# ebeauce/Seismic_BPMF

Hardware: AMD Instinct MI355X
Metric: million network-CC-samples/s (matched filter) (higher is better)
Workload: dtype f32

## Files before the change

### seismic_bpmf_amd/csrc/mf.hip

```cpp
#include "common.h"
#include "context.h"
#include "mf_split_api.h"
#include <system_error>
#include <thread>
#include <chrono>
#include <vector>
#include <mutex>
#include <utility>
#include <cstring>
#include <algorithm>
#include "../../include/bpmf_hip.h"

#include <cstdlib>

namespace bpmf {

typedef float f32x16 __attribute__((ext_vector_type(16)));


__device__ __forceinline__ int2 mf_lag_range(bool any, long long mv_min, long long mv_max, long long step,
                                             long long L, long long N, long long n_corr, int exclusive_last)
{
    int2 r = make_int2(1, 0);
    if (any && N >= L) {
        long long first = mv_min < 0 ? (-mv_min + step - 1) / step : 0;
        long long room = N - L - mv_max;
        if (exclusive_last & 1) room -= 1;
        if (room >= 0) {
            long long last = room / step;
            if (last > n_corr - 1) last = n_corr - 1;
            if (first <= last) r = make_int2((int)first, (int)last);
        }
    }
    return r;
}

__global__ __launch_bounds__(64) void mf_prologue_kernel(const float* __restrict__ tmpl, const int* __restrict__ mv,
                                                         const float* __restrict__ w, int T, int n_ch, long long step,
                                                         long long L, long long N, long long n_corr, int exclusive_last,
                                                         int sqrt_norm, float* __restrict__ e_t, int2* __restrict__ range,
                                                         int4* __restrict__ chan_rec)
{
    const int t = blockIdx.x;
    for (int ch = threadIdx.x; ch < n_ch; ch += 64) {
        const float* x = tmpl + ((size_t)t * n_ch + ch) * (size_t)L;
        float acc = 0.0f;
        for (int l = 0; l < (int)L; ++l) acc = __fmaf_rn(x[l], x[l], acc);
        e_t[(size_t)t * n_ch + ch] = sqrt_norm ? acc : 1.0f / sqrtf(acc);
    }
    __syncthreads();
    if (threadIdx.x != 0) return;
    long long mv_min = 0, mv_max = 0;
    bool any = false, seen = false;
    const bool all_channels = (exclusive_last & 2) != 0;
    int4* rec = chan_rec + (size_t)t * (n_ch + 2);
    int n_used = 0;
    for (int ch = 0; ch < n_ch; ++ch) {
        const float wc = w[(size_t)t * n_ch + ch];
        if (wc == 0.0f && !all_channels) continue;
        long long m = mv[(size_t)t * n_ch + ch];
        if (!seen || m < mv_min) mv_min = m;
        if (!seen || m > mv_max) mv_max = m;
        seen = true;
        if (wc == 0.0f) continue;
        rec[n_used++] = make_int4(ch, (int)m, __float_as_int(wc),
                                  __float_as_int(((volatile const float*)e_t)[(size_t)t * n_ch + ch]));
        any = true;
    }
    rec[n_used] = make_int4(-1, 0, 0, 0);
    rec[n_used + 1] = make_int4(-1, 0, 0, 0);
    range[t] = mf_lag_range(any, mv_min, mv_max, step, L, N, n_corr, exclusive_last);
}

__global__ void mf_csum_local_kernel(const float* __restrict__ data, size_t n_ch, size_t N,
                                     size_t nq, double* __restrict__ local,
                                     double* __restrict__ tot, size_t q_lo, size_t q_cnt)
{
    size_t idx = (size_t)blockIdx.x * blockDim.x + threadIdx.x;
    if (idx >= n_ch * q_cnt) return;
    size_t ch = idx / q_cnt, q = q_lo + idx % q_cnt;
    size_t n0 = q * CSUM_CHUNK;
    size_t n1 = n0 + CSUM_CHUNK < N ? n0 + CSUM_CHUNK : N;
    const float* d = data + ch * N;
    double* lo = local + ch * N;
    double acc = 0.0;
    typedef float f32x4a __attribute__((ext_vector_type(4), aligned(4)));
    typedef double f64x2a __attribute__((ext_vector_type(2), aligned(8)));
    size_t n = n0;
    constexpr int NB = 8;
    f32x4a cur[NB], nxt[NB];
    const size_t nbatch = (n1 - n0) / (4 * NB);
    if (nbatch) {
#pragma unroll
        for (int i = 0; i < NB; ++i) cur[i] = *(const f32x4a*)(d + n + 4 * i);
    }
    for (size_t b = 0; b < nbatch; ++b, n += 4 * NB) {
        if (b + 1 < nbatch) {
#pragma unroll
            for (int i = 0; i < NB; ++i) nxt[i] = *(const f32x4a*)(d + n + 4 * NB + 4 * i);
        }
#pragma unroll
        for (int i = 0; i < NB; ++i) {
            const f32x4a v = cur[i];
            f64x2a o0, o1;
            double x = (double)v[0]; acc = acc + x * x; o0[0] = acc;
            x = (double)v[1]; acc = acc + x * x; o0[1] = acc;
            x = (double)v[2]; acc = acc + x * x; o1[0] = acc;
            x = (double)v[3]; acc = acc + x * x; o1[1] = acc;
            *(f64x2a*)(lo + n + 4 * i) = o0;
            *(f64x2a*)(lo + n + 4 * i + 2) = o1;
        }
#pragma unroll
        for (int i = 0; i < NB; ++i) cur[i] = nxt[i];
    }
    for (; n + 4 <= n1; n += 4) {
        const f32x4a v = *(const f32x4a*)(d + n);
        f64x2a o0, o1;
        double x = (double)v[0]; acc = acc + x * x; o0[0] = acc;
        x = (double)v[1]; acc = acc + x * x; o0[1] = acc;
        x = (double)v[2]; acc = acc + x * x; o1[0] = acc;
        x = (double)v[3]; acc = acc + x * x; o1[1] = acc;
        *(f64x2a*)(lo + n) = o0;
        *(f64x2a*)(lo + n + 2) = o1;
    }
    for (; n < n1; ++n) {
        double v = (double)d[n];
        acc = acc + v * v;
        lo[n] = acc;
    }
    tot[ch * nq + q] = acc;
}

__global__ __launch_bounds__(64) void mf_csum_sequential_kernel(const float* __restrict__ data, size_t N, size_t nq,
                                                                double* __restrict__ local, double* __restrict__ off)
{
    __shared__ float s_in[CSUM_CHUNK];
    __shared__ double s_out[CSUM_CHUNK];
    const size_t ch = blockIdx.x;
    const int lane = threadIdx.x;
    const float* d = data + ch * N;
    double* lo = local + ch * N;
    double acc = 0.0;
    for (size_t q = 0; q < nq; ++q) {
        const size_t n0 = q * CSUM_CHUNK;
        const size_t len = n0 + CSUM_CHUNK < N ? CSUM_CHUNK : N - n0;
        for (size_t i = lane; i < len; i += 64) s_in[i] = d[n0 + i];
        if (lane == 0) off[ch * nq + q] = 0.0;
        __syncthreads();
        if (lane == 0) {
            for (size_t i = 0; i < len; ++i) {
                const double v = (double)s_in[i];
                acc = acc + v * v;
                s_out[i] = acc;
            }
        }
        __syncthreads();
        for (size_t i = lane; i < len; i += 64) lo[n0 + i] = s_out[i];
        __syncthreads();
    }
}

__global__ void mf_csum_offsets_kernel(const double* __restrict__ tot, size_t n_ch, size_t nq,
                                       double* __restrict__ off, size_t q_lo, size_t q_hi)
{
    size_t ch = (size_t)blockIdx.x * blockDim.x + threadIdx.x;
    if (ch >= n_ch) return;
    const double* tr = tot + ch * nq;
    double* orow = off + ch * nq;
    double acc = q_lo ? orow[q_lo - 1] + tr[q_lo - 1] : 0.0;
    size_t q = q_lo;
    for (; q + 16 <= q_hi; q += 16) {
        double v[16];
#pragma unroll
        for (int i = 0; i < 16; ++i) v[i] = tr[q + i];
#pragma unroll
        for (int i = 0; i < 16; ++i) {
            orow[q + i] = acc;
            acc = acc + v[i];
        }
    }
    for (; q < q_hi; ++q) {
        orow[q] = acc;
        acc = acc + tr[q];
    }
}

__global__ void mf_window_energy_kernel(const double* __restrict__ local,
                                        const double* __restrict__ off, size_t n_ch, size_t N,
                                        size_t nq, size_t L, size_t nwin, int sqrt_norm,
                                        float* __restrict__ e_d, size_t w_lo, size_t w_hi)
{
    size_t j = w_lo + (size_t)blockIdx.x * blockDim.x + threadIdx.x;
    size_t ch = blockIdx.y;
    if (j >= w_hi) return;
    const double* lo = local + ch * N;
    const double* of = off + ch * nq;
    size_t nh = j + L - 1;
    double hi = of[nh / CSUM_CHUNK] + lo[nh];
    double low = 0.0;
    if (j > 0) low = of[(j - 1) / CSUM_CHUNK] + lo[j - 1];
    const float e = (float)(hi - low);
    e_d[ch * nwin + j] = sqrt_norm ? e : 1.0f / sqrtf(e);
}


template <bool SQRT_NORM>
__device__ __forceinline__ float mf_cc_of(float num, float nt, float nd)
{
    if constexpr (SQRT_NORM) {
        const float den2 = nt * nd;
        return den2 > 1.0e-6f ? num / sqrtf(den2) : 0.0f;
    } else {
        const float nrm = nt * nd;
        return nrm < MAX_NORM ? num * nrm : 0.0f;
    }
}

constexpr int MF_THREADS = 256;
constexpr int MF_LAGS_PER_WAVE = 1024;
constexpr int MF_LAGS_PER_WG = 4096;
constexpr int MF_REC_TERMINATORS = 12;

typedef float f32x4 __attribute__((ext_vector_type(4)));
typedef float f32x4u __attribute__((ext_vector_type(4), aligned(4)));

__device__ __forceinline__ int mf_pad(int x) { return x + (x >> 4); }

__host__ __device__ inline int mf_kpad(int L) { return (L + 15 + 15) / 16 * 16; }
__host__ __device__ inline int mf_band_len(int L) { return mf_kpad(L) + 16; }
__host__ __device__ inline int mf_window_len(int L) { return MF_LAGS_PER_WG - 16 + mf_kpad(L); }
__host__ __device__ inline int mf_buf_floats(int L)
{
    const int W = mf_window_len(L);
    return mf_band_len(L) + (W + (W >> 4) + 1);
}
__host__ inline size_t mf_lds_bytes(int L) { return ((size_t)2 * mf_buf_floats(L) + 64) * sizeof(float); }

__device__ __forceinline__ bool mf_tile_of_block(unsigned bid, int T, int n_lag_blocks, int& t,
                                                 long long& lag_block)
{
    const unsigned xcd = bid & 7u, i = bid >> 3;
    const unsigned total = (unsigned)n_lag_blocks * (unsigned)T;
    const unsigned per_xcd = (total + 7u) >> 3;
    const unsigned flat = xcd * per_xcd + i;
    t = (int)(flat % (unsigned)T);
    lag_block = (long long)(flat / (unsigned)T);
    return i < per_xcd && flat < total;
}

template <int NR, int STRIDE>
__device__ __forceinline__ void mf_stage_rows(float (&rd)[NR], __amdgpu_buffer_rsrc_t rs,
                                              long long first, int idx)
{
    const unsigned o = (unsigned)((first + idx) * 4);
    if (first >= 0) {
#pragma unroll
        for (int r = 0; r < NR; ++r)
            rd[r] = __builtin_bit_cast(float, __builtin_amdgcn_raw_buffer_load_b32(rs, (int)(o + STRIDE * 4u * r), 0, 0));
    } else {
        unsigned oo = o;
#pragma unroll
        for (int r = 0; r < NR; ++r) {
            asm volatile("" : "+v"(oo));
            rd[r] = __builtin_bit_cast(float, __builtin_amdgcn_raw_buffer_load_b32(rs, (int)oo, 0, 0));
            oo += STRIDE * 4u;
        }
    }
}
template <int NR, int STRIDE>
__device__ __forceinline__ void mf_stage_band(float (&rt)[NR], __amdgpu_buffer_rsrc_t rs, int idx)
{
    int o0 = (idx - 15) * 4;
    asm volatile("" : "+v"(o0));
    rt[0] = __builtin_bit_cast(float, __builtin_amdgcn_raw_buffer_load_b32(rs, o0, 0, 0));
#pragma unroll
    for (int r = 1; r < NR; ++r)
        rt[r] = __builtin_bit_cast(float, __builtin_amdgcn_raw_buffer_load_b32(
                                              rs, idx * 4 + (STRIDE * r - 15) * 4, 0, 0));
}

template <bool NETWORK_SUM, int MAXR, int MAXT, bool STEP1, bool SQRT_NORM = false>
__global__ __launch_bounds__(MF_THREADS, 2) void mf_mfma_kernel(
    const float* __restrict__ tmpl, const int4* __restrict__ chan_rec,
    const float* __restrict__ data, const float* __restrict__ e_d,
    const int2* __restrict__ range, int L, long long N, int T, int n_ch, long long n_corr, int step,
    float* __restrict__ out, int n_lag_blocks, int prio, int lag_block0)
{
    extern __shared__ float smem[];
    const int Kpad = mf_kpad(L);
    const int tp_len = mf_band_len(L);
    const int W = mf_window_len(L);
    const int buf_floats = mf_buf_floats(L);

    const int tid = threadIdx.x;
    const int lane = tid & 63;
    const int wv = tid >> 6;
    const int a = lane & 15;
    const int kq = lane >> 4;

    int t;
    long long lag_block;
    if (!mf_tile_of_block(blockIdx.x, T, n_lag_blocks, t, lag_block)) return;
    lag_block += lag_block0;
    const long long lag0 = lag_block * MF_LAGS_PER_WG;
    const int2 rgi = range[t];
    const int2 rg = make_int2(rgi.x * step, rgi.y * step);
    const long long nwin = N - L + 1;

    f32x4 sum[4];
#pragma unroll
    for (int u = 0; u < 4; ++u) sum[u] = (f32x4){0.0f, 0.0f, 0.0f, 0.0f};

    const bool wg_valid = rg.x <= rg.y && !(lag0 > rg.y || lag0 + MF_LAGS_PER_WG - 1 < rg.x);
    const bool wg_inside = lag0 >= rg.x && lag0 + MF_LAGS_PER_WG - 1 <= rg.y;
    const long long lag_w = lag0 + (long long)wv * MF_LAGS_PER_WAVE + 16 * a + 4 * kq;

    if (wg_valid) {
        const int a_base = 15 - a + kq;
        const int b_base = 1088 * wv + 17 * a + kq;
        const int4* __restrict__ recs = chan_rec + (size_t)t * (n_ch + 2);

        float rd[MAXR], rt[MAXT];
        auto issue_stage = [&](int ch, int mvc) {
            const __amdgpu_buffer_rsrc_t rs_d = __builtin_amdgcn_make_buffer_rsrc(
                (void*)(data + (size_t)ch * (size_t)N), 0, (int)(N * 4), 0x00020000);
            mf_stage_rows<MAXR, MF_THREADS>(rd, rs_d, lag0 + mvc, tid);
            const __amdgpu_buffer_rsrc_t rs_t = __builtin_amdgcn_make_buffer_rsrc(
                (void*)(tmpl + ((size_t)t * n_ch + ch) * (size_t)L), 0, L * 4, 0x00020000);
            mf_stage_band<MAXT, MF_THREADS>(rt, rs_t, tid);
        };
        auto write_stage = [&](float* tp, float* dw) {
#pragma unroll
            for (int r = 0; r < MAXR; ++r) {
                const int x = tid + MF_THREADS * r;
                if (x < W) dw[mf_pad(x)] = rd[r];
            }
#pragma unroll
            for (int r = 0; r < MAXT; ++r) {
                const int x = tid + MF_THREADS * r;
                if (x < tp_len) tp[x] = rt[r];
            }
        };
        int4 rec = recs[0];
        int4 rec1 = recs[1];
        int ri = 0;
        if (rec.x >= 0) issue_stage(rec.x, rec.y);
        int buf = 0;
        while (rec.x >= 0) {
            const int ch = rec.x;
            float* tp = smem + buf * buf_floats;
            float* dw = tp + tp_len;
            write_stage(tp, dw);
            __syncthreads();
            const float w = __int_as_float(rec.z);
            const int mvc = rec.y;
            const float et = __int_as_float(rec.w);
            const int4 rec2 = recs[ri + 2];
            const float* edc = e_d + (size_t)ch * (size_t)nwin;
            f32x4 ed[4];
#pragma unroll
            for (int u = 0; u < 4; ++u) {
                const long long lag = lag_w + 256 * u;
                if (wg_inside || (lag + 3 >= rg.x && lag <= rg.y)) {
                    ed[u] = *(const f32x4u*)(edc + lag + mvc);
                } else {
                    ed[u] = (f32x4){0.0f, 0.0f, 0.0f, 0.0f};
                }
            }
            if (rec1.x >= 0) issue_stage(rec1.x, rec1.y);

            f32x4 acc[4];
#pragma unroll
            for (int u = 0; u < 4; ++u) acc[u] = (f32x4){0.0f, 0.0f, 0.0f, 0.0f};
            const int nq = Kpad >> 4;
            const unsigned a_addr = (unsigned)(size_t)(tp + a_base) ;
            const unsigned b_addr = (unsigned)(size_t)(dw + b_base);
            unsigned ap = a_addr, bp = b_addr;
            float sa[4], sb[4][4];
#define MF_LDS_READ(dst, addr, off) \
    asm volatile("ds_read_b32 %0, %1 offset:%2" : "=v"(dst) : "v"(addr), "n"(off))
#define MF_MFMA(slot, u) \
    acc[u] = __builtin_amdgcn_mfma_f32_16x16x4f32(sa[slot], sb[slot][u], acc[u], 0, 0, 0)
#define MF_REQ(slot, aoff, boff)                                    \
    MF_LDS_READ(sa[slot], ap, (aoff));                               \
    MF_LDS_READ(sb[slot][0], bp, (boff));                            \
    MF_LDS_READ(sb[slot][1], bp, (boff) + 1088);                     \
    MF_LDS_READ(sb[slot][2], bp, (boff) + 2176);                     \
    MF_LDS_READ(sb[slot][3], bp, (boff) + 3264)
#define MF_STEP(cur, req, aoff, boff)                                \
    asm volatile("s_waitcnt lgkmcnt(5)" ::: "memory");               \
    __builtin_amdgcn_sched_barrier(0);                               \
    MF_MFMA(cur, 0);                                                 \
    __builtin_amdgcn_sched_barrier(0);                               \
    MF_LDS_READ(sa[req], ap, (aoff));                                \
    __builtin_amdgcn_sched_barrier(0);                               \
    MF_MFMA(cur, 1);                                                 \
    __builtin_amdgcn_sched_barrier(0);                               \
    MF_LDS_READ(sb[req][0], bp, (boff));                             \
    __builtin_amdgcn_sched_barrier(0);                               \
    MF_MFMA(cur, 2);                                                 \
    __builtin_amdgcn_sched_barrier(0);                               \
    MF_LDS_READ(sb[req][1], bp, (boff) + 1088);                      \
    __builtin_amdgcn_sched_barrier(0);                               \
    MF_MFMA(cur, 3);                                                 \
    __builtin_amdgcn_sched_barrier(0);                               \
    MF_LDS_READ(sb[req][2], bp, (boff) + 2176);                      \
    MF_LDS_READ(sb[req][3], bp, (boff) + 3264);                      \
    __builtin_amdgcn_sched_barrier(0)
            __builtin_amdgcn_sched_barrier(0);
            if (prio) __builtin_amdgcn_s_setprio(0);
            MF_REQ(0, 0, 0);
            MF_REQ(1, 16, 16);
            for (int q = 0; q < nq; ++q) {
                MF_STEP(0, 2, 32, 32);
                MF_STEP(1, 3, 48, 48);
                MF_STEP(2, 0, 64, 68);
                MF_STEP(3, 1, 80, 84);
                ap += 64;
                bp += 68;
            }
            asm volatile("s_waitcnt lgkmcnt(0)" ::: "memory");
            __builtin_amdgcn_sched_barrier(0);
            if (prio == 1) __builtin_amdgcn_s_setprio(1);
            else if (prio == 2) __builtin_amdgcn_s_setprio(2);
            else if (prio == 3) __builtin_amdgcn_s_setprio(3);
#undef MF_LDS_READ
#undef MF_MFMA
#undef MF_REQ
#undef MF_STEP

            if (NETWORK_SUM && STEP1 && wg_inside) {
#pragma unroll
                for (int u = 0; u < 4; ++u) {
#pragma unroll
                    for (int r = 0; r < 4; ++r) {
                        const float cc = mf_cc_of<SQRT_NORM>(acc[u][r], et, ed[u][r]);
                        sum[u][r] = __fmaf_rn(w, cc, sum[u][r]);
                    }
                }
            } else {
#pragma unroll
            for (int u = 0; u < 4; ++u) {
#pragma unroll
                for (int r = 0; r < 4; ++r) {
                    const long long lag = lag_w + 256 * u + r;
                    const bool ok = lag >= rg.x && lag <= rg.y && (STEP1 || (unsigned)lag % (unsigned)step == 0);
                    float cc = 0.0f;
                    if (ok) {
                        cc = mf_cc_of<SQRT_NORM>(acc[u][r], et, ed[u][r]);
                        if (!NETWORK_SUM)
                            out[((size_t)t * n_corr + (STEP1 ? lag : (long long)((unsigned)lag / (unsigned)step))) * n_ch + ch] = cc;
                    }
                    if (NETWORK_SUM) sum[u][r] = __fmaf_rn(w, cc, sum[u][r]);
                }
            }
            }
            rec = rec1;
            rec1 = rec2;
            ++ri;
            buf ^= 1;
        }
    }
    if (NETWORK_SUM) {
#pragma unroll
        for (int u = 0; u < 4; ++u) {
            const long long lag = lag_w + 256 * u;
            float* dst = out + (size_t)t * n_corr + lag;
            if (STEP1 && lag + 3 < n_corr) {
                *(f32x4u*)dst = sum[u];
            } else {
#pragma unroll
                for (int r = 0; r < 4; ++r) {
                    const unsigned smp = (unsigned)(lag + r);
                    const long long i = STEP1 ? (long long)smp : (long long)(smp / (unsigned)step);
                    if ((STEP1 || smp % (unsigned)step == 0) && i < n_corr) out[(size_t)t * n_corr + i] = sum[u][r];
                }
            }
        }
    }
}

template <bool SQRT_NORM>
__device__ __forceinline__ int2 mf_fused_prologue(const float* __restrict__ tmpl, const int* __restrict__ mv,
                                                  const float* __restrict__ w, int t, int n_ch, long long step, int L,
                                                  long long N, long long n_corr, int exclusive_last,
                                                  int4* l_rec, int* l_part)
{
    const int tid = threadIdx.x, lane = tid & 63, wv = tid >> 6;
    float wc = 0.0f, nt = 0.0f;
    int m = 0;
    bool used = false;
    if (tid < n_ch) {
        wc = w[(size_t)t * n_ch + tid];
        used = !(wc == 0.0f);
    }
    const bool all_channels = (exclusive_last & 2) != 0;
    if (tid < n_ch && (used || all_channels)) m = mv[(size_t)t * n_ch + tid];
    if (used) {
        const float* x = tmpl + ((size_t)t * n_ch + tid) * (size_t)L;
        float acc = 0.0f;
        int l = 0;
        for (; l + 16 <= L; l += 16) {
            const f32x4u v0 = *(const f32x4u*)(x + l), v1 = *(const f32x4u*)(x + l + 4);
            const f32x4u v2 = *(const f32x4u*)(x + l + 8), v3 = *(const f32x4u*)(x + l + 12);
#pragma unroll
            for (int i = 0; i < 4; ++i) acc = __fmaf_rn(v0[i], v0[i], acc);
#pragma unroll
            for (int i = 0; i < 4; ++i) acc = __fmaf_rn(v1[i], v1[i], acc);
#pragma unroll
            for (int i = 0; i < 4; ++i) acc = __fmaf_rn(v2[i], v2[i], acc);
#pragma unroll
            for (int i = 0; i < 4; ++i) acc = __fmaf_rn(v3[i], v3[i], acc);
        }
        for (; l < L; ++l) acc = __fmaf_rn(x[l], x[l], acc);
        nt = SQRT_NORM ? acc : 1.0f / sqrtf(acc);
    }
    const unsigned long long mask = __ballot(used);
    const int idx = __popcll(mask & ((1ull << lane) - 1ull));
    const bool ranged = used || (all_channels && tid < n_ch);
    int mn = ranged ? m : 0x7fffffff, mx = ranged ? m : (int)0x80000000;
#pragma unroll
    for (int o = 32; o > 0; o >>= 1) {
        mn = min(mn, __shfl_xor(mn, o));
        mx = max(mx, __shfl_xor(mx, o));
    }
    if (lane == 0) {
        l_part[wv] = __popcll(mask);
        l_part[4 + wv] = mn;
        l_part[8 + wv] = mx;
    }
    __syncthreads();
    int base = 0, n_used = 0, mv_min_i = 0x7fffffff, mv_max_i = (int)0x80000000;
#pragma unroll
    for (int i = 0; i < 4; ++i) {
        const int c = l_part[i];
        if (i < wv) base += c;
        n_used += c;
        mv_min_i = min(mv_min_i, l_part[4 + i]);
        mv_max_i = max(mv_max_i, l_part[8 + i]);
    }
    if (used) l_rec[base + idx] = make_int4(tid, m, __float_as_int(wc), __float_as_int(nt));
    if (tid < MF_REC_TERMINATORS) l_rec[n_used + tid] = make_int4(-1, 0, 0, 0);
    __syncthreads();
    return mf_lag_range(n_used > 0, mv_min_i, mv_max_i, step, L, N, n_corr, exclusive_last);
}

#ifdef BPMF_PHASE_CYCLES
__device__ unsigned long long g_mf_phase[8];
#define MF_PHASE_DECL unsigned long long ph_last_ = 0, ph_acc_[4] = {0, 0, 0, 0}; unsigned ph_n_ = 0;
#define MF_PHASE_START() asm volatile("s_memtime %0\n\ts_waitcnt lgkmcnt(0)" : "=s"(ph_last_) :: "memory")
#define MF_PHASE(i)                                                                                \
    do {                                                                                           \
        unsigned long long t_;                                                                     \
        asm volatile("s_memtime %0\n\ts_waitcnt lgkmcnt(0)" : "=s"(t_) :: "memory");              \
        ph_acc_[i] += t_ - ph_last_;                                                               \
        ph_last_ = t_;                                                                             \
    } while (0)
#else
#define MF_PHASE_DECL
#define MF_PHASE_START() do {} while (0)
#define MF_PHASE(i) do {} while (0)
#endif

template <bool NETWORK_SUM, int MAXR, int MAXT, bool STEP1, int NTILE = 4, bool SQRT_NORM = false, bool FUSED = false, bool CSPLIT = false>
__global__ __launch_bounds__(MF_THREADS, 4) void mf_mfma_wave_kernel(
    const float* __restrict__ tmpl, const int4* __restrict__ chan_rec,
    const float* __restrict__ data, const float* __restrict__ e_d,
    const int2* __restrict__ range, int L, long long N, int T, int n_ch, long long n_corr, int step,
    float* __restrict__ out, int n_lag_blocks, int prio, const int* __restrict__ mv,
    const float* __restrict__ wts, int exclusive_last, int lag_block0)
{
    extern __shared__ float smem[];
    const int Kpad = mf_kpad(L);
    const int tp_len = mf_band_len(L);
    static_assert(NTILE == 4 || NTILE == 2 || NTILE == 1, "tiles per wave");
    static_assert(!CSPLIT || (NTILE == 1 && FUSED && NETWORK_SUM && STEP1), "channel split: the tiny-problem variant only");
    constexpr int LAGS_W = 256 * NTILE, LAGS_WG = CSPLIT ? LAGS_W : 4 * LAGS_W;
    constexpr int REC_STRIDE = CSPLIT ? 4 : 1;
    const int Ww = LAGS_W - 16 + Kpad;
    constexpr bool FULLW = NTILE < 4;
    const int Wbuf = FULLW ? 64 * MAXR : Ww;
    const int wave_floats = tp_len + (Wbuf + 2 * (Wbuf >> 4) + 2 + 63) / 64 * 64 + 64;

    const int tid = threadIdx.x;
    const int lane = tid & 63;
    const int wv = __builtin_amdgcn_readfirstlane(tid >> 6);
    const int a = lane & 15;
    const int kq = lane >> 4;

    int t;
    long long lag_block;
    if (!mf_tile_of_block(blockIdx.x, T, n_lag_blocks, t, lag_block)) return;
    lag_block += lag_block0;
    int2 rgi;
    int4* l_rec = nullptr;
    if constexpr (FUSED) {
        int* l_part = (int*)(smem + 4 * wave_floats + 64);
        l_rec = (int4*)(l_part + 16);
        const int2 r = mf_fused_prologue<SQRT_NORM>(tmpl, mv, wts, t, n_ch, (long long)step, L, N, n_corr, exclusive_last,
                                                    l_rec, l_part);
        rgi = make_int2(__builtin_amdgcn_readfirstlane(r.x), __builtin_amdgcn_readfirstlane(r.y));
    } else {
        rgi = range[t];
    }
    float* exch = nullptr;
    int n_used = 0;
    if constexpr (CSPLIT) {
        const int* l_part = (const int*)(smem + 4 * wave_floats + 64);
        n_used = l_part[0] + l_part[1] + l_part[2] + l_part[3];
        exch = (float*)(l_rec + n_ch + MF_REC_TERMINATORS);
    }
    const long long lag0 = lag_block * LAGS_WG + (CSPLIT ? 0 : (long long)wv * LAGS_W);
    const int2 rg = make_int2(rgi.x * step, rgi.y * step);
    const long long nwin = N - L + 1;

    f32x4 sum[NTILE];
#pragma unroll
    for (int u = 0; u < NTILE; ++u) sum[u] = (f32x4){0.0f, 0.0f, 0.0f, 0.0f};

    const bool wave_valid = rg.x <= rg.y && !(lag0 > rg.y || lag0 + LAGS_W - 1 < rg.x);
    const bool wave_inside = lag0 >= rg.x && lag0 + LAGS_W - 1 <= rg.y;
    const long long lag_w = lag0 + 16 * a + 4 * kq;
    MF_PHASE_DECL

    if (wave_valid) {
        float* tp = smem + wv * wave_floats;
        float* dw = tp + tp_len;
        const int a_base = 15 - a + kq;
        const int b_base = 18 * a + kq;
        const int4* __restrict__ recs = FUSED ? nullptr : chan_rec + (size_t)t * (n_ch + 2);
        auto ld_rec = [&](int i) -> int4 {
            if constexpr (FUSED) {
                const int4 v = l_rec[i];
                return make_int4(__builtin_amdgcn_readfirstlane(v.x), __builtin_amdgcn_readfirstlane(v.y),
                                 __builtin_amdgcn_readfirstlane(v.z), __builtin_amdgcn_readfirstlane(v.w));
            } else {
                return recs[i];
            }
        };

        float rd[MAXR], rt[MAXT];
        auto issue_stage = [&](int ch, int mvc) {
            const __amdgpu_buffer_rsrc_t rs_d = __builtin_amdgcn_make_buffer_rsrc(
                (void*)(data + (size_t)ch * (size_t)N), 0, (int)(N * 4), 0x00020000);
            mf_stage_rows<MAXR, 64>(rd, rs_d, lag0 + mvc, lane);
            const __amdgpu_buffer_rsrc_t rs_t = __builtin_amdgcn_make_buffer_rsrc(
                (void*)(tmpl + ((size_t)t * n_ch + ch) * (size_t)L), 0, L * 4, 0x00020000);
            mf_stage_band<MAXT, 64>(rt, rs_t, lane);
        };
        const int rd_chunks = (Ww + 63) >> 6, rt_chunks = (tp_len + 63) >> 6;
        auto write_stage = [&]() {
            if constexpr (FULLW) {
#pragma unroll
                for (int r = 0; r < MAXT; ++r) tp[lane + 64 * r] = rt[r];
#pragma unroll
                for (int r = 0; r < MAXR; ++r) {
                    const int x = lane + 64 * r;
                    dw[x + 2 * (x >> 4)] = rd[r];
                }
                return;
            }
#define MF_WT(r) case (r) + 1: if constexpr ((r) < MAXT) tp[lane + 64 * ((r) < MAXT ? (r) : 0)] = rt[(r) < MAXT ? (r) : 0]; [[fallthrough]];
            switch (rt_chunks) {
                MF_WT(4) MF_WT(3) MF_WT(2) MF_WT(1) MF_WT(0)
                default: break;
            }
#undef MF_WT
#define MF_WD(r) case (r) + 1: if constexpr ((r) < MAXR) { const int x = lane + 64 * (r); dw[x + 2 * (x >> 4)] = rd[(r) < MAXR ? (r) : 0]; } [[fallthrough]];
            switch (rd_chunks) {
                MF_WD(19) MF_WD(18) MF_WD(17) MF_WD(16) MF_WD(15) MF_WD(14) MF_WD(13) MF_WD(12) MF_WD(11) MF_WD(10)
                MF_WD(9) MF_WD(8) MF_WD(7) MF_WD(6) MF_WD(5) MF_WD(4) MF_WD(3) MF_WD(2) MF_WD(1) MF_WD(0)
                default: break;
            }
#undef MF_WD
        };

        int4 rec = ld_rec(CSPLIT ? wv : 0);
        int4 rec1 = ld_rec(CSPLIT ? wv + REC_STRIDE : 1);
        int ri = CSPLIT ? wv : 0;
        if (rec.x >= 0) issue_stage(rec.x, rec.y);
        MF_PHASE_START();
        while (rec.x >= 0) {
            const int ch = rec.x;
            write_stage();
            MF_PHASE(0);
            const float w = __int_as_float(rec.z);
            const int mvc = rec.y;
            const float et = __int_as_float(rec.w);
            const int4 rec2 = ld_rec(ri + 2 * REC_STRIDE);
            const float* edc = e_d + (size_t)ch * (size_t)nwin;
            f32x4 ed[NTILE];
            if (wave_inside) {
#pragma unroll
                for (int u = 0; u < NTILE; ++u) ed[u] = *(const f32x4u*)(edc + lag_w + 256 * u + mvc);
            } else {
#pragma unroll
                for (int u = 0; u < NTILE; ++u) {
                    const long long lag = lag_w + 256 * u;
                    if (lag + 3 >= rg.x && lag <= rg.y) {
                        ed[u] = *(const f32x4u*)(edc + lag + mvc);
                    } else {
                        ed[u] = (f32x4){0.0f, 0.0f, 0.0f, 0.0f};
                    }
                }
            }
            if (rec1.x >= 0) issue_stage(rec1.x, rec1.y);
            MF_PHASE(1);

            f32x4 acc[NTILE];
#pragma unroll
            for (int u = 0; u < NTILE; ++u) acc[u] = (f32x4){0.0f, 0.0f, 0.0f, 0.0f};
            const int nq = Kpad >> 4;
            unsigned ap = (unsigned)(size_t)(tp + a_base), bp = (unsigned)(size_t)(dw + b_base);
            float sa[4], sb[4][NTILE];
#define MF_LDS_READ(dst, addr, off) \
    asm volatile("ds_read_b32 %0, %1 offset:%2" : "=v"(dst) : "v"(addr), "n"(off))
#define MF_MFMA(slot, u) \
    acc[u] = __builtin_amdgcn_mfma_f32_16x16x4f32(sa[slot], sb[slot][u], acc[u], 0, 0, 0)
#define MF_REQ(slot, aoff, boff)                                                    \
    MF_LDS_READ(sa[slot], ap, (aoff));                                               \
    MF_LDS_READ(sb[slot][0], bp, (boff));                                            \
    if constexpr (NTILE > 1) MF_LDS_READ(sb[slot][1 % NTILE], bp, (boff) + 1152);    \
    if constexpr (NTILE > 2) MF_LDS_READ(sb[slot][2 % NTILE], bp, (boff) + 2304);    \
    if constexpr (NTILE > 2) MF_LDS_READ(sb[slot][3 % NTILE], bp, (boff) + 3456)
#define MF_STEP(cur, req, aoff, boff)                                                \
    asm volatile("s_waitcnt lgkmcnt(%0)" :: "n"(NTILE + 1) : "memory");              \
    __builtin_amdgcn_sched_barrier(0);                                               \
    MF_MFMA(cur, 0);                                                                 \
    __builtin_amdgcn_sched_barrier(0);                                               \
    MF_LDS_READ(sa[req], ap, (aoff));                                                \
    __builtin_amdgcn_sched_barrier(0);                                               \
    if constexpr (NTILE > 1) { MF_MFMA(cur, 1 % NTILE); __builtin_amdgcn_sched_barrier(0); } \
    MF_LDS_READ(sb[req][0], bp, (boff));                                             \
    __builtin_amdgcn_sched_barrier(0);                                               \
    if constexpr (NTILE > 2) { MF_MFMA(cur, 2 % NTILE); __builtin_amdgcn_sched_barrier(0); } \
    if constexpr (NTILE > 1) { MF_LDS_READ(sb[req][1 % NTILE], bp, (boff) + 1152); __builtin_amdgcn_sched_barrier(0); } \
    if constexpr (NTILE > 2) { MF_MFMA(cur, 3 % NTILE); __builtin_amdgcn_sched_barrier(0); } \
    if constexpr (NTILE > 2) { MF_LDS_READ(sb[req][2 % NTILE], bp, (boff) + 2304); MF_LDS_READ(sb[req][3 % NTILE], bp, (boff) + 3456); } \
    __builtin_amdgcn_sched_barrier(0)
            __builtin_amdgcn_sched_barrier(0);
            if (prio) __builtin_amdgcn_s_setprio(0);
            MF_REQ(0, 0, 0);
            MF_REQ(1, 16, 16);
            for (int q = 0; q < nq; ++q) {
                MF_STEP(0, 2, 32, 32);
                MF_STEP(1, 3, 48, 48);
                MF_STEP(2, 0, 64, 72);
                MF_STEP(3, 1, 80, 88);
                ap += 64;
                bp += 72;
            }
            asm volatile("s_waitcnt lgkmcnt(0)" ::: "memory");
            __builtin_amdgcn_sched_barrier(0);
            if (prio == 1) __builtin_amdgcn_s_setprio(1);
            else if (prio == 2) __builtin_amdgcn_s_setprio(2);
            else if (prio == 3) __builtin_amdgcn_s_setprio(3);
#undef MF_LDS_READ
#undef MF_MFMA
#undef MF_REQ
#undef MF_STEP
            MF_PHASE(2);
            if constexpr (CSPLIT) {
                f32x4 c4;
#pragma unroll
                for (int r = 0; r < 4; ++r) {
                    const long long lag = lag_w + r;
                    const bool ok = wave_inside || (lag >= rg.x && lag <= rg.y);
                    c4[r] = ok ? mf_cc_of<SQRT_NORM>(acc[0][r], et, ed[0][r]) : 0.0f;
                }
                *(f32x4*)(exch + ri * 256 + 16 * a + 4 * kq) = c4;
            } else if (NETWORK_SUM && STEP1 && wave_inside) {
#pragma unroll
                for (int u = 0; u < NTILE; ++u) {
#pragma unroll
                    for (int r = 0; r < 4; ++r) {
                        const float cc = mf_cc_of<SQRT_NORM>(acc[u][r], et, ed[u][r]);
                        sum[u][r] = __fmaf_rn(w, cc, sum[u][r]);
                    }
                }
            } else {
#pragma unroll
            for (int u = 0; u < NTILE; ++u) {
#pragma unroll
                for (int r = 0; r < 4; ++r) {
                    const long long lag = lag_w + 256 * u + r;
                    const bool ok = lag >= rg.x && lag <= rg.y && (STEP1 || (unsigned)lag % (unsigned)step == 0);
                    float cc = 0.0f;
                    if (ok) {
                        cc = mf_cc_of<SQRT_NORM>(acc[u][r], et, ed[u][r]);
                        if (!NETWORK_SUM)
                            out[((size_t)t * n_corr + (STEP1 ? lag : (long long)((unsigned)lag / (unsigned)step))) * n_ch + ch] = cc;
                    }
                    if (NETWORK_SUM) sum[u][r] = __fmaf_rn(w, cc, sum[u][r]);
                }
            }
            }
            rec = rec1;
            rec1 = rec2;
            ri += REC_STRIDE;
            MF_PHASE(3);
#ifdef BPMF_PHASE_CYCLES
            ++ph_n_;
#endif
        }
    }
    if constexpr (CSPLIT) {
        __syncthreads();
        const long long lag = lag0 + tid;
        float s = 0.0f;
        if (wave_valid) {
            for (int i = 0; i < n_used; ++i) s = __fmaf_rn(__int_as_float(l_rec[i].z), exch[i * 256 + tid], s);
        }
        if (lag < n_corr) out[(size_t)t * n_corr + lag] = s;
    } else if (NETWORK_SUM) {
#pragma unroll
        for (int u = 0; u < NTILE; ++u) {
            const long long lag = lag_w + 256 * u;
            float* dst = out + (size_t)t * n_corr + lag;
            if (STEP1 && lag + 3 < n_corr) {
                *(f32x4u*)dst = sum[u];
            } else {
#pragma unroll
                for (int r = 0; r < 4; ++r) {
                    const unsigned smp = (unsigned)(lag + r);
                    const long long i = STEP1 ? (long long)smp : (long long)(smp / (unsigned)step);
                    if ((STEP1 || smp % (unsigned)step == 0) && i < n_corr) out[(size_t)t * n_corr + i] = sum[u][r];
                }
            }
        }
    }
#ifdef BPMF_PHASE_CYCLES
    if (lane == 0 && ph_n_) {
        for (int i = 0; i < 4; ++i) atomicAdd(&g_mf_phase[i], ph_acc_[i]);
        atomicAdd(&g_mf_phase[4], (unsigned long long)ph_n_);
        atomicAdd(&g_mf_phase[5], 1ull);
    }
#endif
}

template <bool NETWORK_SUM, bool SQRT_NORM = false>
__global__ __launch_bounds__(256) void mf_direct_kernel(
    const float* __restrict__ tmpl, const int* __restrict__ mv, const float* __restrict__ wgt,
    const float* __restrict__ data, const float* __restrict__ e_t,
    const float* __restrict__ e_d, const int2* __restrict__ range, long long step, int L,
    long long N, int n_ch, long long n_corr, float* __restrict__ out,
    const double* __restrict__ cs_local = nullptr, const double* __restrict__ cs_off = nullptr, long long nq = 0)
{
    const long long i = (long long)blockIdx.x * blockDim.x + threadIdx.x;
    const int t = blockIdx.y;
    if (i >= n_corr) return;
    const int2 rg = range[t];
    const bool ok = i >= rg.x && i <= rg.y;
    const long long nwin = N - L + 1;
    float sum = 0.0f;
    if (ok) {
        for (int ch = 0; ch < n_ch; ++ch) {
            const float w = wgt[(size_t)t * n_ch + ch];
            if (w == 0.0f) continue;
            const long long j = i * step + mv[(size_t)t * n_ch + ch];
            const float* tp = tmpl + ((size_t)t * n_ch + ch) * (size_t)L;
            const float* d = data + (size_t)ch * (size_t)N + j;
            float num = 0.0f;
            for (int l = 0; l < L; ++l) num = __fmaf_rn(tp[l], d[l], num);
            float cc = 0.0f;
            if constexpr (SQRT_NORM) {
                float et = 0.0f;
                for (int l = 0; l < L; ++l) et = __fmaf_rn(tp[l], tp[l], et);
                const double* lo = cs_local + (size_t)ch * (size_t)N;
                const double* of = cs_off + (size_t)ch * (size_t)nq;
                const long long nh = j + L - 1;
                const double hi = of[nh / CSUM_CHUNK] + lo[nh];
                const double low = j > 0 ? of[(j - 1) / CSUM_CHUNK] + lo[j - 1] : 0.0;
                const float den2 = et * (float)(hi - low);
                if (den2 > 1.0e-6f) cc = num / sqrtf(den2);
            } else {
                const float nrm = e_t[(size_t)t * n_ch + ch] * e_d[(size_t)ch * nwin + j];
                if (nrm < MAX_NORM) cc = num * nrm;
            }
            if (NETWORK_SUM)
                sum = __fmaf_rn(w, cc, sum);
            else
                out[((size_t)t * n_corr + i) * n_ch + ch] = cc;
        }
    }
    if (NETWORK_SUM) out[(size_t)t * n_corr + i] = sum;
}

struct MfWorkspace {
    double* local;
    double* tot;
    double* off;
    float* e_d;
    float* e_t;
    int2* range;
    int4* chan_rec;
    void* sp_day;
    void* sp_batch;
    size_t bytes;
};

static MfWorkspace mf_carve(void* base, size_t L, size_t N, size_t T, size_t n_ch)
{
    MfWorkspace ws;
    const size_t nq = (N + CSUM_CHUNK - 1) / CSUM_CHUNK;
    const size_t nwin = N >= L ? N - L + 1 : 0;
    char* p = (char*)base;
    size_t o = 0;
    ws.local = (double*)(p + o); o += align_up(n_ch * N * sizeof(double), 256);
    ws.tot = (double*)(p + o);   o += align_up(n_ch * nq * sizeof(double), 256);
    ws.off = (double*)(p + o);   o += align_up(n_ch * nq * sizeof(double), 256);
    o += 256;
    ws.e_d = (float*)(p + o);    o += align_up(n_ch * nwin * sizeof(float) + 64, 256);
    const bool split16 = option(OPT_MF_SPLIT16) != 0;
    ws.sp_day = nullptr;
    ws.sp_batch = nullptr;
    if (split16) { ws.sp_day = p + o; o += align_up(sp::day_region_bytes(N, n_ch), 256); }
    ws.e_t = (float*)(p + o);    o += align_up(T * n_ch * sizeof(float), 256);
    ws.range = (int2*)(p + o);   o += align_up(T * sizeof(int2), 256);
    ws.chan_rec = (int4*)(p + o); o += align_up(T * (n_ch + 2) * sizeof(int4), 256);
    if (split16) { ws.sp_batch = p + o; o += align_up(sp::batch_region_bytes(T, n_ch, L), 256); }
    ws.bytes = o;
    return ws;
}

static int mf_check_sizes(size_t step, size_t L, size_t N, size_t T, size_t S, size_t C,
                          size_t n_corr)
{
    if (step == 0 || L == 0 || T == 0 || S == 0 || C == 0) {
        set_error("matched filter: zero-sized dimension (step=%zu L=%zu T=%zu S=%zu C=%zu)", step,
                  L, T, S, C);
        return -1;
    }
    if (N < L) {
        set_error("matched filter: data (N=%zu) shorter than the templates (L=%zu)", N, L);
        return -1;
    }
    if (n_corr != (N - L) / step + 1) {
        set_error("matched filter: n_corr=%zu but (N-L)/step+1=%zu", n_corr, (N - L) / step + 1);
        return -1;
    }
    if (N > 0x7fffffffull || T * S * C > 0x7fffffffull || L > 0x7fffffffull) {
        set_error("matched filter: dimension exceeds the int32 index range");
        return -1;
    }
    return 0;
}

struct MfLaunch {
    long long off_lo = 0, off_hi = -1;
    bool first_piece = true;
};

static std::mutex g_split_days_mutex;
struct SplitDay { const void* data; size_t N, n_ch; };
static std::vector<std::pair<const void*, SplitDay>> g_split_days;
static void split_day_note(const void* ws_base, const void* data, size_t N, size_t n_ch, bool with_split)
{
    std::lock_guard<std::mutex> g(g_split_days_mutex);
    for (size_t i = 0; i < g_split_days.size(); ++i)
        if (g_split_days[i].first == ws_base) { g_split_days.erase(g_split_days.begin() + i); break; }
    if (with_split) {
        if (g_split_days.size() >= 64) g_split_days.erase(g_split_days.begin());
        g_split_days.push_back({ws_base, {data, N, n_ch}});
    }
}
static bool split_day_known(const void* ws_base, const void* data, size_t N, size_t n_ch)
{
    std::lock_guard<std::mutex> g(g_split_days_mutex);
    for (auto& e : g_split_days)
        if (e.first == ws_base) return e.second.data == data && e.second.N == N && e.second.n_ch == n_ch;
    return false;
}

enum MfFamily { MF_DIRECT = 0, MF_WORKGROUP = 1, MF_WAVE = 2, MF_SPLIT16 = 3 };
enum MfRefusal { MF_ACCEPTED = 0, MF_GRID_TOO_LARGE = 1, MF_TOO_MANY_TEMPLATES = 2 };
static const char* const MF_REFUSAL_TEXT[] = {"", "grid too large", "generic kernel supports at most 65535 templates per call"};

struct MfVariant {
    int family, refusal;
    int maxr, maxt;
    int ntile;
    bool fused, csplit;
    bool sqrt_norm, step1, prologue;
    size_t lags_wg, lds, grid;
};

constexpr int MF_WAVE_MAXT = 5;
constexpr int mf_wave_maxr(int ntile) { return ntile == 4 ? 20 : (ntile == 2 ? 12 : 8); }
static size_t mf_grid(size_t T, size_t n_blocks) { return 8 * ((T * n_blocks + 7) / 8); }

static MfVariant mf_choose(size_t step, size_t L, size_t N, size_t T, size_t n_ch, size_t n_corr, int network_sum,
                           int flags, bool ranged)
{
    MfVariant v = {};
    v.sqrt_norm = option(OPT_MF_COMPAT_SQRT_NORM) != 0;
    v.step1 = step == 1;
    v.prologue = true;
    const size_t n_offsets = (n_corr - 1) * step + 1;
    const size_t n_lag_blocks = (n_offsets + MF_LAGS_PER_WG - 1) / MF_LAGS_PER_WG;
    const int need_r = (mf_window_len((int)L) + MF_THREADS - 1) / MF_THREADS;
    const int need_t = (mf_band_len((int)L) + MF_THREADS - 1) / MF_THREADS;
    const bool mfma = step <= (size_t)option(OPT_MF_MAX_MFMA_STEP) && !(flags & BPMF_MF_FORCE_DIRECT) && need_r <= 24 &&
                      need_t <= 9 && T * (n_lag_blocks + 8) < 0x7fffffffull && N < ((size_t)1 << 30) - 8192;
    if (!mfma) {
        v.family = MF_DIRECT;
        v.lags_wg = 256;
        v.grid = (n_corr + 255) / 256 * T;
        if (T > 65535) v.refusal = MF_TOO_MANY_TEMPLATES;
        return v;
    }
    constexpr size_t SP_MIN_BLOCKS = 128;
    const size_t sp_blocks = (n_offsets + sp::LAGS_PER_WG - 1) / sp::LAGS_PER_WG;
    const bool sp_small = option(OPT_MF_SPLIT16) == 1 && T * sp_blocks < SP_MIN_BLOCKS;
    if (option(OPT_MF_SPLIT16) != 0 && sp::usable(L, N) && !sp_small) {
        v.family = MF_SPLIT16;
        v.lags_wg = sp::LAGS_PER_WG;
        v.grid = mf_grid(T, sp_blocks);
        return v;
    }
    if (option(OPT_MF_WAVE_KERNEL) == 0 || mf_kpad((int)L) > 272) {
        v.family = MF_WORKGROUP;
        v.maxr = need_r <= 20 && need_t <= 5 ? 20 : 24;
        v.maxt = v.maxr == 20 ? 5 : 9;
        v.lags_wg = MF_LAGS_PER_WG;
        v.lds = mf_lds_bytes((int)L);
        v.grid = mf_grid(T, n_lag_blocks);
        return v;
    }
    v.family = MF_WAVE;
    const size_t waves4 = T * n_lag_blocks * 4;
    v.ntile = waves4 >= 8192 ? 4 : (waves4 >= 1024 ? 2 : 1);
    const long forced = option(OPT_MF_TILES_PER_WAVE);
    if (forced == 1 || forced == 2 || forced == 4) v.ntile = (int)forced;
    v.maxr = mf_wave_maxr(v.ntile);
    v.maxt = MF_WAVE_MAXT;
    v.fused = v.ntile < 4 && n_ch <= 256 && option(OPT_MF_FUSED_PROLOGUE) != 0;
    v.prologue = !v.fused;
    const long csplit_max = option(OPT_MF_CHANNEL_SPLIT);
    v.csplit = v.ntile == 1 && v.fused && network_sum && v.step1 && n_ch <= 32 && !ranged && csplit_max > 0 &&
               waves4 * 4 <= (size_t)csplit_max;
    v.lags_wg = v.csplit ? (size_t)256 : (size_t)4 * 256 * v.ntile;
    const size_t n_blocks_w = (n_offsets + v.lags_wg - 1) / v.lags_wg;
    if (T * (n_blocks_w + 8) >= 0x7fffffffull) v.refusal = MF_GRID_TOO_LARGE;
    v.grid = mf_grid(T, n_blocks_w);
    const int Wbuf = v.ntile < 4 ? 64 * v.maxr : 256 * v.ntile - 16 + mf_kpad((int)L);
    v.lds = (size_t)4 * (mf_band_len((int)L) + (Wbuf + 2 * (Wbuf >> 4) + 2 + 63) / 64 * 64 + 64) * sizeof(float) + 256 +
            (v.fused ? 64 + (n_ch + MF_REC_TERMINATORS) * sizeof(int4) : 0) +
            (v.csplit ? n_ch * 256 * sizeof(float) : 0);
    return v;
}

}

using namespace bpmf;

extern "C" size_t bpmf_mf_workspace_bytes(size_t L, size_t N, size_t T, size_t S, size_t C)
{
    return mf_carve(nullptr, L, N, T, S * C).bytes;
}

static int mf_prepare_range(const float* d_data, size_t L, size_t N, size_t n_ch, const MfWorkspace& ws,
                            hipStream_t stream, size_t samp_lo, size_t samp_hi)
{
    const size_t nq = (N + CSUM_CHUNK - 1) / CSUM_CHUNK;
    const size_t nwin = N - L + 1;
    const size_t q_lo = samp_lo / CSUM_CHUNK, q_hi = (samp_hi + CSUM_CHUNK - 1) / CSUM_CHUNK;
    if (q_hi <= q_lo) return 0;
    {
        size_t n = n_ch * (q_hi - q_lo);
        mf_csum_local_kernel<<<dim3((unsigned)((n + 63) / 64)), dim3(64), 0, stream>>>(
            d_data, n_ch, N, nq, ws.local, ws.tot, q_lo, q_hi - q_lo);
        BPMF_LAUNCH_CHECK();
    }
// ... 431 lines not shown
```

Before: 4380.

## Use 128-bit buffer loads and vectorized LDS stores for interior data staging

For the full-width non-fused tile configuration, when the whole data window lies inside the trace, each lane loads 16 contiguous bytes per row with b128 buffer loads instead of scalar per-lane loads. It then writes them into the padded LDS layout with paired 64-bit stores. The network-sum epilogue gains a wave-uniform fast path that skips the per-element MAX_NORM select when no lane exceeds it. The scalar LDS store addressing is also simplified to a precomputed base with constant strides. The cost is more code paths and register pressure, and the permuted lane-to-sample mapping must match what the MFMA reads expect.

```diff
diff --git a/seismic_bpmf_amd/csrc/mf.hip b/seismic_bpmf_amd/csrc/mf.hip
--- a/seismic_bpmf_amd/csrc/mf.hip
+++ b/seismic_bpmf_amd/csrc/mf.hip
@@ -223,6 +223,7 @@
 
 typedef float f32x4 __attribute__((ext_vector_type(4)));
 typedef float f32x4u __attribute__((ext_vector_type(4), aligned(4)));
+typedef float f32x2 __attribute__((ext_vector_type(2)));
 
 __device__ __forceinline__ int mf_pad(int x) { return x + (x >> 4); }
 
@@ -640,12 +641,36 @@
         };
 
         float rd[MAXR], rt[MAXT];
+        constexpr bool WIDE = NTILE == 4 && !FUSED && !CSPLIT && MAXR == 20 && MAXT == 5;
+        bool wide = false;
+        const bool lane5 = 1024 + 4 * lane < Ww;
+        const int off5 = lane * 16 + (lane5 ? 4096 : 0);
+        float* const wq = dw + 4 * lane + 2 * (lane >> 2);
+        float* const wq5 = wq + (lane5 ? 4 * 288 : 0);
         auto issue_stage = [&](int ch, int mvc) {
             const __amdgpu_buffer_rsrc_t rs_d = __builtin_amdgcn_make_buffer_rsrc(
                 (void*)(data + (size_t)ch * (size_t)N), 0, (int)(N * 4), 0x00020000);
-            mf_stage_rows<MAXR, 64>(rd, rs_d, lag0 + mvc, lane);
             const __amdgpu_buffer_rsrc_t rs_t = __builtin_amdgcn_make_buffer_rsrc(
                 (void*)(tmpl + ((size_t)t * n_ch + ch) * (size_t)L), 0, L * 4, 0x00020000);
+            if constexpr (WIDE) {
+                const long long first = lag0 + mvc;
+                wide = first >= 0 && first + Ww <= N;
+                if (wide) {
+                    const __amdgpu_buffer_rsrc_t rs_w = __builtin_amdgcn_make_buffer_rsrc(
+                        (void*)(data + (size_t)ch * (size_t)N + first), 0, Ww * 4, 0x00020000);
+                    asm volatile("; mf.interior loads begin" ::: "memory");
+#pragma unroll
+                    for (int r = 0; r < 5; ++r) {
+                        const f32x4 v = __builtin_bit_cast(f32x4, r < 4 ? __builtin_amdgcn_raw_buffer_load_b128(rs_w, lane * 16, 1024 * r, 0)
+                                                                        : __builtin_amdgcn_raw_buffer_load_b128(rs_w, off5, 0, 0));
+                        rd[4 * r] = v[0]; rd[4 * r + 1] = v[1]; rd[4 * r + 2] = v[2]; rd[4 * r + 3] = v[3];
+                    }
+                    mf_stage_band<MAXT, 64>(rt, rs_t, lane);
+                    asm volatile("; mf.interior loads end" ::: "memory");
+                    return;
+                }
+            }
+            mf_stage_rows<MAXR, 64>(rd, rs_d, lag0 + mvc, lane);
             mf_stage_band<MAXT, 64>(rt, rs_t, lane);
         };
         const int rd_chunks = (Ww + 63) >> 6, rt_chunks = (tp_len + 63) >> 6;
@@ -660,13 +685,29 @@
                 }
                 return;
             }
+            if constexpr (WIDE) {
+                if (wide) {
+                    asm volatile("; mf.interior stores begin" ::: "memory");
+#pragma unroll
+                    for (int r = MAXT - 1; r >= 0; --r) tp[lane + 64 * r] = rt[r];
+#pragma unroll
+                    for (int r = 0; r < 5; ++r) {
+                        float* q = r < 4 ? wq + 288 * r : wq5;
+                        *(f32x2*)q = (f32x2){rd[4 * r], rd[4 * r + 1]};
+                        *(f32x2*)(q + 2) = (f32x2){rd[4 * r + 2], rd[4 * r + 3]};
+                    }
+                    asm volatile("; mf.interior stores end" ::: "memory");
+                    return;
+                }
+            }
 #define MF_WT(r) case (r) + 1: if constexpr ((r) < MAXT) tp[lane + 64 * ((r) < MAXT ? (r) : 0)] = rt[(r) < MAXT ? (r) : 0]; [[fallthrough]];
             switch (rt_chunks) {
                 MF_WT(4) MF_WT(3) MF_WT(2) MF_WT(1) MF_WT(0)
                 default: break;
             }
 #undef MF_WT
-#define MF_WD(r) case (r) + 1: if constexpr ((r) < MAXR) { const int x = lane + 64 * (r); dw[x + 2 * (x >> 4)] = rd[(r) < MAXR ? (r) : 0]; } [[fallthrough]];
+            float* we = dw + lane + 2 * (lane >> 4);
+#define MF_WD(r) case (r) + 1: if constexpr ((r) < MAXR) we[72 * (r)] = rd[(r) < MAXR ? (r) : 0]; [[fallthrough]];
             switch (rd_chunks) {
                 MF_WD(19) MF_WD(18) MF_WD(17) MF_WD(16) MF_WD(15) MF_WD(14) MF_WD(13) MF_WD(12) MF_WD(11) MF_WD(10)
                 MF_WD(9) MF_WD(8) MF_WD(7) MF_WD(6) MF_WD(5) MF_WD(4) MF_WD(3) MF_WD(2) MF_WD(1) MF_WD(0)
@@ -769,6 +810,48 @@
                     c4[r] = ok ? mf_cc_of<SQRT_NORM>(acc[0][r], et, ed[0][r]) : 0.0f;
                 }
                 *(f32x4*)(exch + ri * 256 + 16 * a + 4 * kq) = c4;
+            } else if constexpr (WIDE && NETWORK_SUM) {
+                f32x4 cc[NTILE];
+                if (STEP1 && wave_inside) {
+                    bool plain = false;
+                    if constexpr (!SQRT_NORM) {
+                        unsigned top = 0;
+#pragma unroll
+                        for (int u = 0; u < NTILE; ++u) {
+#pragma unroll
+                            for (int r = 0; r < 4; ++r) top = max(top, __float_as_uint(et * ed[u][r]));
+                        }
+                        plain = __builtin_amdgcn_ballot_w64(top >= __builtin_bit_cast(unsigned, MAX_NORM)) == 0;
+                    }
+                    if (plain) {
+#pragma unroll
+                        for (int u = 0; u < NTILE; ++u) {
+#pragma unroll
+                            for (int r = 0; r < 4; ++r) cc[u][r] = acc[u][r] * (et * ed[u][r]);
+                        }
+                    } else {
+#pragma unroll
+                        for (int u = 0; u < NTILE; ++u) {
+#pragma unroll
+                            for (int r = 0; r < 4; ++r) cc[u][r] = mf_cc_of<SQRT_NORM>(acc[u][r], et, ed[u][r]);
+                        }
+                    }
+                } else {
+#pragma unroll
+                    for (int u = 0; u < NTILE; ++u) {
+#pragma unroll
+                        for (int r = 0; r < 4; ++r) {
+                            const long long lag = lag_w + 256 * u + r;
+                            const bool ok = lag >= rg.x && lag <= rg.y && (STEP1 || (unsigned)lag % (unsigned)step == 0);
+                            cc[u][r] = ok ? mf_cc_of<SQRT_NORM>(acc[u][r], et, ed[u][r]) : 0.0f;
+                        }
+                    }
+                }
+#pragma unroll
+                for (int u = 0; u < NTILE; ++u) {
+#pragma unroll
+                    for (int r = 0; r < 4; ++r) sum[u][r] = __fmaf_rn(w, cc[u][r], sum[u][r]);
+                }
             } else if (NETWORK_SUM && STEP1 && wave_inside) {
 #pragma unroll
                 for (int u = 0; u < NTILE; ++u) {
```

After: 4413, median of 6. No clear change (+0.8%).
